# dcharatan/pixelsplat

Measured on NVIDIA H100. Metric: rendered views/sec fwd+bwd @256x256, 3 gauss/px, higher is better.
Workload: dtype f32

## Files before the change

pixelsplat_b200/csrc/ps_common.cuh:

```cuda
#pragma once
#include <cuda_runtime.h>
#include <stdint.h>

#include "../../include/pixelsplat_b200.h"

namespace ps {

constexpr int kTile = PS_TILE;
constexpr int kTilePixels = kTile * kTile;

struct Geom {
    float *depth;
    int32_t *radii;
    float2 *xy;
    float4 *conic_opacity;
    float4 *rgb;
    ushort4 *rect;
    uint8_t *clamped;
    uint32_t *tile_count;
    uint32_t *tile_start;
    uint32_t *tile_cursor;
    long long *n_instances;
    uint32_t *vis_pairs;
    float4 *cull;
};

struct ImageState {
    float *final_T;
    uint32_t *n_contrib;
    float *color;
    float4 *run_state;
    float *depth_image;
    float *run_depth;
};

// ... 66 lines not shown
    return 1.0f;
}

__device__ __forceinline__ float2 cull_extent(float a, float c, float o) {
    if (!(a > 0.0f) || !(c > 0.0f) || !(o <= 3.0e38f)) return make_float2(3.0e38f, 3.0e38f);
    if (!(o * 255.0f >= 1.0f - 1e-3f)) return make_float2(-3.0e38f, -3.0e38f);
    const float tau2 = 2.0f * (__logf(fmaxf(o * 255.0f, 1.0f)) + 0.01f);
    return make_float2(sqrtf(tau2 * a) * 1.001f + 0.01f, sqrtf(tau2 * c) * 1.001f + 0.01f);
}

constexpr uint32_t kLivePosLimit = 1u << 24;

__device__ __forceinline__ uint32_t tile_block_mask(const float4 &cr, int x0, int y0) {
    const float xl = cr.x - cr.z, xh = cr.x + cr.z, yl = cr.y - cr.w, yh = cr.y + cr.w;
    uint32_t xm = 0, m = 0;
#pragma unroll
    for (int bx = 0; bx < 2; ++bx)
        xm |= ((xh >= (float)(x0 + 8 * bx)) && (xl <= (float)(x0 + 8 * bx + 7))) ? 1u << bx : 0u;
#pragma unroll
    for (int by = 0; by < 4; ++by)
        m |= ((yh >= (float)(y0 + 4 * by)) && (yl <= (float)(y0 + 4 * by + 3))) ? xm << (2 * by) : 0u;
    return m;
}

void set_error(const char *fmt, ...);

enum Mark { kMarkFwdStart = 0, kMarkPreprocess, kMarkScatter, kMarkSort, kMarkCompositeFwd,
            kMarkBwdStart, kMarkBwdZero, kMarkCompositeBwd, kMarkPreprocessBwd, kNumMarks };
void mark(int id, cudaStream_t st);
void count_launch();

bool first_use_on_device(unsigned long long &mask);

#define PS_CUDA_CHECK(expr)                                                              \
    do {                                                                                 \
        cudaError_t _e = (expr);                                                         \
        if (_e != cudaSuccess) {                                                         \
            ps::set_error("%s failed: %s (%s:%d)", #expr, cudaGetErrorString(_e), __FILE__, __LINE__); \
            return PS_ERR_CUDA;                                                          \
        }                                                                                \
    } while (0)

#define PS_LAUNCH_CHECK(name)                                                            \
    do {                                                                                 \
        cudaError_t _e = cudaGetLastError();                                             \
        if (_e != cudaSuccess) {                                                         \
            ps::set_error("launch of %s failed: %s", name, cudaGetErrorString(_e));      \
            return PS_ERR_CUDA;                                                          \
        }                                                                                \
        ps::count_launch();                                                              \
    } while (0)

int launch_preprocess(const Dims &d, const Inputs &in, const Geom &g, cudaStream_t st);
int launch_sh_color(const Dims &d, const Inputs &in, const Geom &g, cudaStream_t st);
int launch_binning(const Dims &d, const Geom &g, unsigned long long *keys,
                   unsigned long long *keys_alt, int sort_impl, int segment_hint, cudaEvent_t scanned,
                   cudaStream_t st);
int launch_composite_forward(const Dims &d, const Inputs &in, const Geom &g,
                             const unsigned long long *keys, const uint2 *live, const ImageState &img,
                             float *out_color, const LossEpilogue &loss, const HitLists &hl, float *loss_partials,
                             cudaStream_t st);
int launch_composite_backward(const Dims &d, const Inputs &in, const Geom &g,
                              const unsigned long long *keys, const uint2 *live, const ImageState &img,
                              const float *d_color, const float *d_depth, const ViewGrads &vg,
                              const ViewGrads *records, const LossEpilogue &loss, const HitLists &hl,
                              cudaStream_t st);
// ... 17 lines not shown
```

pixelsplat_b200/csrc/raster_api.cu:

```cuda
#include <cstdarg>
#include <atomic>
#include <cstdio>
#include <cstring>
#include <mutex>

#include "ps_common.cuh"

namespace ps {

static thread_local char g_error[512] = "";

void set_error(const char *fmt, ...) {
    va_list ap;
    va_start(ap, fmt);
    vsnprintf(g_error, sizeof(g_error), fmt, ap);
    va_end(ap);
}

static bool g_timing = false;
static cudaEvent_t g_events[kNumMarks];
static bool g_events_ready = false;
static std::atomic<unsigned long long> g_launches{0};

void count_launch() { g_launches.fetch_add(1, std::memory_order_relaxed); }

static std::mutex g_once_mutex;

bool first_use_on_device(unsigned long long &mask) {
    int dev = 0;
    cudaGetDevice(&dev);
    const unsigned long long bit = 1ull << (dev & 63);
    std::lock_guard<std::mutex> lock(g_once_mutex);
    if (mask & bit) return false;
    mask |= bit;
    return true;
}

void mark(int id, cudaStream_t st) {
    if (!g_timing) return;
    if (!g_events_ready) {
        for (int i = 0; i < kNumMarks; ++i) cudaEventCreate(&g_events[i]);
        g_events_ready = true;
    }
    cudaEventRecord(g_events[id], st);
}

struct SideCtx {
    cudaStream_t side = nullptr;
    cudaEvent_t fork = nullptr, join = nullptr;
    cudaEvent_t scanned = nullptr, copied = nullptr;
    std::mutex enqueue;
};
static SideCtx g_side_ctx[64];

static int side_ready(SideCtx *&ctx) {
    int dev = 0;
    PS_CUDA_CHECK(cudaGetDevice(&dev));
    ctx = &g_side_ctx[dev & 63];
    std::lock_guard<std::mutex> lock(g_once_mutex);
    if (ctx->side) return PS_OK;
    PS_CUDA_CHECK(cudaStreamCreateWithFlags(&ctx->side, cudaStreamNonBlocking));
    PS_CUDA_CHECK(cudaEventCreateWithFlags(&ctx->fork, cudaEventDisableTiming));
    PS_CUDA_CHECK(cudaEventCreateWithFlags(&ctx->join, cudaEventDisableTiming));
    PS_CUDA_CHECK(cudaEventCreateWithFlags(&ctx->scanned, cudaEventDisableTiming));
    PS_CUDA_CHECK(cudaEventCreateWithFlags(&ctx->copied, cudaEventDisableTiming));
    return PS_OK;
}

// ... 457 lines not shown
```

pixelsplat_b200/csrc/raster_binning.cu:

```cuda
#include <cub/device/device_segmented_radix_sort.cuh>

#include "ps_common.cuh"

namespace ps {

constexpr int kScanThreads = 1024;

__global__ void __launch_bounds__(kScanThreads)
k_tile_scan(int n, const uint32_t *__restrict__ count, uint32_t *__restrict__ start,
            uint32_t *__restrict__ cursor, long long *__restrict__ n_instances) {
    __shared__ uint32_t warp_sums[32];
    __shared__ unsigned long long carry_s;
    const int tid = threadIdx.x, lane = tid & 31, warp = tid >> 5;
    if (tid == 0) carry_s = 0;
    __syncthreads();
    uint32_t cmax = 0;
    for (int base = 0; base < n; base += kScanThreads) {
        const int i = base + tid;
        const uint32_t c = i < n ? count[i] : 0u;
        cmax = max(cmax, c);
        uint32_t x = c;
#pragma unroll
        for (int o = 1; o < 32; o <<= 1) {
            const uint32_t y = __shfl_up_sync(0xffffffffu, x, o);
// ... 1 lines not shown
        }
        if (lane == 31) warp_sums[warp] = x;
        __syncthreads();
        if (warp == 0) {
            uint32_t w = warp_sums[lane];
#pragma unroll
            for (int o = 1; o < 32; o <<= 1) {
                const uint32_t y = __shfl_up_sync(0xffffffffu, w, o);
                if (lane >= o) w += y;
            }
            warp_sums[lane] = w;
        }
        __syncthreads();
        const unsigned long long carry = carry_s;
        const uint32_t warp_off = warp ? warp_sums[warp - 1] : 0u;
        const unsigned long long excl = carry + warp_off + (x - c);
        if (i < n) {
            const uint32_t e = excl > 0xffffffffull ? 0xffffffffu : (uint32_t)excl;
            start[i] = e;
            cursor[i] = e;
        }
        __syncthreads();
        if (tid == kScanThreads - 1) carry_s = carry + warp_sums[31];
        __syncthreads();
    }
    if (tid == 0) *n_instances = (long long)carry_s;
    cmax = __reduce_max_sync(0xffffffffu, cmax);
    if (lane == 0 && cmax) atomicMax(reinterpret_cast<unsigned long long *>(n_instances + 1), (unsigned long long)cmax);
}

constexpr int kScatterThreads = 256;
constexpr int kScatterMaxSmemTiles = 8192;

__global__ void __launch_bounds__(kScatterThreads)
k_scatter(Dims d, Geom geo, unsigned long long *__restrict__ keys, int use_smem) {
    extern __shared__ uint32_t s_scatter[];
    if (*geo.n_instances > d.capacity) return;
    const int vid = blockIdx.y;
    const int g = blockIdx.x * kScatterThreads + threadIdx.x;
    uint32_t *cnt = s_scatter, *base = s_scatter + d.tiles;
    uint32_t *cur = geo.tile_cursor + (size_t)vid * d.tiles;
    const size_t vg = (size_t)vid * d.P + g;
    const bool vis = g < d.P && geo.radii[vg] > 0;
    ushort4 r = make_ushort4(0, 0, 0, 0);
    unsigned long long key = 0;
    if (vis) {
        r = geo.rect[vg];
        key = ((unsigned long long)__float_as_uint(geo.depth[vg]) << 32) | (uint32_t)g;
    }
    if (!use_smem) {
        for (int ty = r.y; ty < r.w; ++ty)
            for (int tx = r.x; tx < r.z; ++tx) keys[atomicAdd(&cur[ty * d.gx + tx], 1u)] = key;
        return;
    }
    for (int i = threadIdx.x; i < d.tiles; i += kScatterThreads) cnt[i] = 0;
    __syncthreads();
    for (int ty = r.y; ty < r.w; ++ty)
        for (int tx = r.x; tx < r.z; ++tx) atomicAdd(&cnt[ty * d.gx + tx], 1u);
    __syncthreads();
    for (int i = threadIdx.x; i < d.tiles; i += kScatterThreads) {
        const uint32_t c = cnt[i];
        if (c) { base[i] = atomicAdd(&cur[i], c); cnt[i] = 0; }
    }
    __syncthreads();
    for (int ty = r.y; ty < r.w; ++ty)
        for (int tx = r.x; tx < r.z; ++tx) {
            const int t = ty * d.gx + tx;
            keys[base[t] + atomicAdd(&cnt[t], 1u)] = key;
        }
}

template <int THREADS>
__device__ void bitonic_sort_smem(unsigned long long *s_keys, int n_pad) {
    constexpr int kWarps = THREADS / 32;
    const int lane = threadIdx.x & 31, warp = threadIdx.x >> 5;
    const int chunk = max(n_pad / kWarps, 2);
    const int warps_used = n_pad / chunk;
    const int half = n_pad >> 1;
    for (int k = 2; k <= n_pad; k <<= 1) {
        int j = k >> 1;
        const bool had_global = j >= chunk;
        for (; j >= chunk; j >>= 1) {
            for (int t = threadIdx.x; t < half; t += THREADS) {
                const int i = 2 * t - (t & (j - 1));
                const int p = i + j;
                const unsigned long long a = s_keys[i], b = s_keys[p];
                const bool up = (i & k) == 0;
                if ((a > b) == up) { s_keys[i] = b; s_keys[p] = a; }
            }
            __syncthreads();
        }
        if (warp < warps_used) {
            const int base = warp * chunk;
            for (; j > 0; j >>= 1) {
                for (int t = lane; t < (chunk >> 1); t += 32) {
                    const int i = base + 2 * t - (t & (j - 1));
                    const int p = i + j;
                    const unsigned long long a = s_keys[i], b = s_keys[p];
                    const bool up = (i & k) == 0;
                    if ((a > b) == up) { s_keys[i] = b; s_keys[p] = a; }
                }
                __syncwarp();
// ... 202 lines not shown
    if (sm.misc[3]) {
        int n_pad = 2;
        while (n_pad < n) n_pad <<= 1;
        for (int i = n + tid; i < n_pad; i += kSortThreads) A[i] = ~0ull;
        __syncthreads();
        bitonic_sort_smem<kSortThreads>(A, n_pad);
    }
    for (int i = tid; i < n; i += kSortThreads) keys[s0 + i] = A[i];
    write_live_list(d, geo, A, n, seg, live, sm);
}

__global__ void __launch_bounds__(kSortThreads)
k_live_lists(Dims d, Geom geo, const unsigned long long *__restrict__ keys, unsigned long long *__restrict__ keys_alt) {
    __shared__ SortSmem sm;
    if (*geo.n_instances > d.capacity) return;
    const int seg = blockIdx.x;
    const uint32_t s0 = geo.tile_start[seg];
    write_live_list(d, geo, keys + s0, (int)geo.tile_count[seg], seg, reinterpret_cast<uint2 *>(keys_alt + s0), sm);
}

int launch_binning(const Dims &d, const Geom &g, unsigned long long *keys,
                   unsigned long long *keys_alt, int sort_impl, int segment_hint, cudaEvent_t scanned,
                   cudaStream_t st) {
    const int n_seg = d.S * d.V * d.tiles;
    k_tile_scan<<<1, kScanThreads, 0, st>>>(n_seg, g.tile_count, g.tile_start, g.tile_cursor, g.n_instances);
    PS_LAUNCH_CHECK("k_tile_scan");
    if (scanned) PS_CUDA_CHECK(cudaEventRecord(scanned, st));
    const int use_smem = d.tiles <= kScatterMaxSmemTiles;
    static unsigned long long scatter_attr_devices = 0;
    if (first_use_on_device(scatter_attr_devices)) {
        PS_CUDA_CHECK(cudaFuncSetAttribute(k_scatter, cudaFuncAttributeMaxDynamicSharedMemorySize,
                                           (int)(2 * sizeof(uint32_t) * kScatterMaxSmemTiles)));
    }
    dim3 sgrid((d.P + kScatterThreads - 1) / kScatterThreads, d.S * d.V);
    k_scatter<<<sgrid, kScatterThreads, use_smem ? 2 * sizeof(uint32_t) * d.tiles : 0, st>>>(d, g, keys, use_smem);
    PS_LAUNCH_CHECK("k_scatter");
    mark(kMarkScatter, st);

    int id_bits = 1;
    while ((1ll << id_bits) < d.P) ++id_bits;

    if (sort_impl == 1) {
        size_t temp = 0;
        cub::DoubleBuffer<unsigned long long> db(keys, keys_alt);
        PS_CUDA_CHECK(cub::DeviceSegmentedRadixSort::SortKeys(nullptr, temp, db, (int)d.capacity, n_seg,
                                                              g.tile_start, g.tile_cursor, 0, 64, st));
        void *tmp = nullptr;
        PS_CUDA_CHECK(cudaMallocAsync(&tmp, temp, st));
        PS_CUDA_CHECK(cub::DeviceSegmentedRadixSort::SortKeys(tmp, temp, db, (int)d.capacity, n_seg,
                                                              g.tile_start, g.tile_cursor, 0, 64, st));
        if (db.Current() != keys)
            PS_CUDA_CHECK(cudaMemcpyAsync(keys, db.Current(), sizeof(unsigned long long) * (size_t)d.capacity,
                                          cudaMemcpyDeviceToDevice, st));
        PS_CUDA_CHECK(cudaFreeAsync(tmp, st));
        k_live_lists<<<n_seg, kSortThreads, 0, st>>>(d, g, keys, keys_alt);
        PS_LAUNCH_CHECK("k_live_lists");
        return PS_OK;
    }

    int cap = 2048;
    if (segment_hint > 0) {
        const long long want = (long long)segment_hint + segment_hint / 4;
        while (cap < want && cap < 8192) cap <<= 1;
    }
    static unsigned long long battr_devices = 0;
    if (first_use_on_device(battr_devices)) {
        PS_CUDA_CHECK(cudaFuncSetAttribute(k_tile_sort, cudaFuncAttributeMaxDynamicSharedMemorySize,
// ... 9 lines not shown
```

pixelsplat_b200/csrc/raster_preprocess.cu:

```cuda
#include "ps_common.cuh"
#include "raster_math.cuh"

namespace ps {

constexpr int kPreThreads = 128;

__device__ __forceinline__ void warp_append(bool flag, uint32_t value, uint32_t *list, long long *counter, int lane) {
    const unsigned m = __ballot_sync(0xffffffffu, flag);
    if (m == 0u) return;
    const int leader = __ffs(m) - 1;
    unsigned long long base = 0;
    if (lane == leader)
        base = atomicAdd(reinterpret_cast<unsigned long long *>(counter), (unsigned long long)__popc(m));
    base = __shfl_sync(0xffffffffu, base, leader);
    if (flag) list[base + __popc(m & ((1u << lane) - 1u))] = value;
}

__global__ void __launch_bounds__(kPreThreads)
k_preprocess(Dims d, Inputs in, Geom geo, int use_smem_hist) {
    extern __shared__ uint32_t s_hist[];
    const int hist_n = d.V * d.tiles;
    const int scene = blockIdx.y;
    const int lane = threadIdx.x & 31;
    const int g = blockIdx.x * kPreThreads + threadIdx.x;
    const bool live = g < d.P;
    if (use_smem_hist) {
        for (int i = threadIdx.x; i < hist_n; i += kPreThreads) s_hist[i] = 0;
        __syncthreads();
    }
    const size_t sg = (size_t)scene * d.P + (live ? g : 0);
    float mx0 = 0.0f, my0 = 0.0f, mz0 = 0.0f, opacity = 0.0f;
    if (live) {
        mx0 = in.means[3 * sg + 0]; my0 = in.means[3 * sg + 1]; mz0 = in.means[3 * sg + 2];
        opacity = in.opac[sg];
    }
    const float *covp = in.cov + sg * (d.cov_layout == PS_COV_TRIU6 ? 6 : 9);
    float cov_raw[6];
    {
        float tmp[6] = {0.0f, 0.0f, 0.0f, 0.0f, 0.0f, 0.0f};
        if (live) load_cov6(covp, d.cov_layout, 1.0f, tmp);
#pragma unroll
        for (int i = 0; i < 6; ++i) cov_raw[i] = tmp[i];
    }

    for (int v = 0; v < d.V; ++v) {
        const int vid = scene * d.V + v;
        const size_t vg = (size_t)vid * d.P + (live ? g : 0);
        const float *__restrict__ vm = in.view + 16 * vid;
        const float *__restrict__ pm = in.proj + 16 * vid;
        const float sc = in.scale ? in.scale[vid] : 1.0f;
        const float px = in.scale ? mx0 * sc : mx0;
        const float py = in.scale ? my0 * sc : my0;
        const float pz = in.scale ? mz0 * sc : mz0;
        bool vis = live;
        float vz = 0.0f;
        if (vis) {
            geo.radii[vg] = 0;
            vz = vm[2] * px + vm[6] * py + vm[10] * pz + vm[14];
            vis = !(vz <= 0.2f);
        }
        if (vis) {
            const float hx = pm[0] * px + pm[4] * py + pm[8] * pz + pm[12];
            const float hy = pm[1] * px + pm[5] * py + pm[9] * pz + pm[13];
            const float hw = pm[3] * px + pm[7] * py + pm[11] * pz + pm[15];
            const float p_w = 1.0f / (hw + 0.0000001f);
            const float projx = hx * p_w, projy = hy * p_w;
            const float tanfovx = in.tanfov[2 * vid], tanfovy = in.tanfov[2 * vid + 1];
            const float focal_x = (float)d.W / (2.0f * tanfovx);
            const float focal_y = (float)d.H / (2.0f * tanfovy);
            float s6[6];
            {
                const float sc2 = sc * sc;
#pragma unroll
                for (int i = 0; i < 6; ++i) s6[i] = in.scale ? cov_raw[i] * sc2 : cov_raw[i];
            }
            Cov2D cv;
            compute_cov2d(px, py, pz, s6, vm, focal_x, focal_y, tanfovx, tanfovy, cv);
            const float det = cv.a * cv.c - cv.b * cv.b;
            vis = !(det == 0.0f);
            if (vis) {
                const float det_inv = 1.0f / det;
                const float mid = 0.5f * (cv.a + cv.c);
                const float sq = sqrtf(fmaxf(0.1f, mid * mid - det));
                const float lambda1 = mid + sq, lambda2 = mid - sq;
                const float my_radius = ceilf(3.0f * sqrtf(fmaxf(lambda1, lambda2)));
                const float pixx = ((projx + 1.0f) * (float)d.W - 1.0f) * 0.5f;
                const float pixy = ((projy + 1.0f) * (float)d.H - 1.0f) * 0.5f;
                const int r = (int)my_radius;
                const float rf = (float)r;
                const int minx = min(d.gx, max(0, (int)((pixx - rf) / (float)kTile)));
                const int miny = min(d.gy, max(0, (int)((pixy - rf) / (float)kTile)));
                const int maxx = min(d.gx, max(0, (int)((pixx + rf + (float)(kTile - 1)) / (float)kTile)));
                const int maxy = min(d.gy, max(0, (int)((pixy + rf + (float)(kTile - 1)) / (float)kTile)));
                vis = (maxx - minx) * (maxy - miny) != 0;
                if (vis) {
                    geo.depth[vg] = vz;
                    geo.radii[vg] = r;
                    geo.xy[vg] = make_float2(pixx, pixy);
                    geo.conic_opacity[vg] = make_float4(cv.c * det_inv, -cv.b * det_inv, cv.a * det_inv, opacity);
                    {
                        const float2 ext = cull_extent(cv.a, cv.c, opacity);
                        geo.cull[vg] = make_float4(pixx, pixy, ext.x, ext.y);
                    }
                    geo.rect[vg] = make_ushort4((unsigned short)minx, (unsigned short)miny,
                                                (unsigned short)maxx, (unsigned short)maxy);
                    if (d.M == 0) {
                        const float *__restrict__ col = in.sh + sg * 3;
                        const float dv = d.depth_mode ? depth_value(d.depth_mode, vz, in.scale, in.near_far, vid) : 0.0f;
                        geo.rgb[vg] = make_float4(col[0], col[1], col[2], dv);
                        geo.clamped[vg] = 0;
                    }
                    for (int ty = miny; ty < maxy; ++ty)
                        for (int tx = minx; tx < maxx; ++tx) {
                            const int t = ty * d.gx + tx;
                            if (use_smem_hist) atomicAdd(&s_hist[v * d.tiles + t], 1u);
                            else atomicAdd(&geo.tile_count[(size_t)vid * d.tiles + t], 1u);
                        }
                }
            }
        }
        warp_append(vis, (uint32_t)vg, geo.vis_pairs, geo.n_instances + 2, lane);
    }
    if (use_smem_hist) {
        __syncthreads();
        uint32_t *dst = geo.tile_count + (size_t)scene * d.V * d.tiles;
        for (int i = threadIdx.x; i < hist_n; i += kPreThreads) {
            const uint32_t c = s_hist[i];
            if (c) atomicAdd(&dst[i], c);
        }
    }
}

constexpr int kShThreads = 128;

__global__ void __launch_bounds__(kShThreads)
k_sh_color(Dims d, Inputs in, Geom geo, int row_stride) {
    extern __shared__ float s_rows[];
    const long long n = geo.n_instances[2];
    const int lane = threadIdx.x & 31, warp = threadIdx.x >> 5;
    const long long i0 = ((long long)blockIdx.x * kShThreads) + warp * 32;
    if (i0 >= n) return;
    const long long i = i0 + lane;
    const bool live = i < n;
    const uint32_t vg = live ? geo.vis_pairs[i] : 0u;
    const uint32_t vid = vg / (uint32_t)d.P, g = vg - vid * (uint32_t)d.P;
    const uint32_t scene = vid / (uint32_t)d.V;
    const size_t sg = (size_t)scene * d.P + g;
    const int sh_n = 3 * d.M;
    float *wrows = s_rows + (size_t)warp * 32 * row_stride;
    gather_rows_async(in.sh, (unsigned long long)sg, __ballot_sync(0xffffffffu, live), sh_n, wrows, row_stride, lane);
    const float sc = in.scale ? in.scale[vid] : 1.0f;
    const float m0 = in.means[3 * sg + 0], m1 = in.means[3 * sg + 1], m2 = in.means[3 * sg + 2];
    const float px = in.scale ? m0 * sc : m0, py = in.scale ? m1 * sc : m1, pz = in.scale ? m2 * sc : m2;
    const float cx = in.campos[3 * vid], cy = in.campos[3 * vid + 1], cz = in.campos[3 * vid + 2];
    const float ddx = px - cx, ddy = py - cy, ddz = pz - cz;
    const float len = sqrtf(ddx * ddx + ddy * ddy + ddz * ddz);
    const float x = ddx / len, y = ddy / len, z = ddz / len;
    gather_rows_wait();
    if (!live) return;
    const float *row = wrows + lane * row_stride;
    float acc[3] = {0.0f, 0.0f, 0.0f};
    const int M = d.M, layout = d.sh_layout;
    const float3 sa = sh_arg(d.sh_basis, x, y, z);
    const uint32_t flip = sh_flip_mask(d.sh_basis);
    sh_for_each(d.deg, sa.x, sa.y, sa.z, [&](int k, float Yk, float, float, float) {
        const float Y = sh_sign(flip, k, Yk);
#pragma unroll
        for (int ch = 0; ch < 3; ++ch) {
            const float c = row[sh_index(layout, M, k, ch)];
            acc[ch] = k == 0 ? Y * c : acc[ch] + Y * c;
        }
    });
    float rgb[3];
    uint8_t clamp_bits = 0;
#pragma unroll
    for (int ch = 0; ch < 3; ++ch) {
        const float a = acc[ch] + 0.5f;
        if (a < 0.0f) clamp_bits |= (uint8_t)(1u << ch);
        rgb[ch] = fmaxf(a, 0.0f);
    }
    const float dv = d.depth_mode ? depth_value(d.depth_mode, geo.depth[vg], in.scale, in.near_far, (int)vid) : 0.0f;
    geo.rgb[vg] = make_float4(rgb[0], rgb[1], rgb[2], dv);
    geo.clamped[vg] = clamp_bits;
}

int launch_sh_color(const Dims &d, const Inputs &in, const Geom &g, cudaStream_t st) {
    if (d.M == 0) return PS_OK;
    const int row_stride = (3 * d.M) | 1;
    const size_t smem = sizeof(float) * kShThreads * row_stride;
    static unsigned long long attr_devices = 0;
    if (first_use_on_device(attr_devices)) {
        PS_CUDA_CHECK(cudaFuncSetAttribute(k_sh_color, cudaFuncAttributeMaxDynamicSharedMemorySize, 64 * 1024));
    }
    const long long pairs = (long long)d.S * d.V * d.P;
    k_sh_color<<<(unsigned)((pairs + kShThreads - 1) / kShThreads), kShThreads, smem, st>>>(d, in, g, row_stride);
    PS_LAUNCH_CHECK("k_sh_color");
    return PS_OK;
}

int launch_preprocess(const Dims &d, const Inputs &in, const Geom &g, cudaStream_t st) {
    PS_CUDA_CHECK(cudaMemsetAsync(g.tile_count, 0, sizeof(uint32_t) * (size_t)d.S * d.V * d.tiles, st));
    PS_CUDA_CHECK(cudaMemsetAsync(g.n_instances, 0, 4 * sizeof(long long), st));
    const size_t hist_bytes = sizeof(uint32_t) * (size_t)d.V * d.tiles;
    const int use_smem = hist_bytes <= 32 * 1024;
    dim3 grid((d.P + kPreThreads - 1) / kPreThreads, d.S);
    k_preprocess<<<grid, kPreThreads, use_smem ? hist_bytes : 0, st>>>(d, in, g, use_smem);
    PS_LAUNCH_CHECK("k_preprocess");
    return PS_OK;
}

}
```

pixelsplat_b200/csrc/raster_preprocess_bwd.cu:

```cuda
#include "ps_common.cuh"
#include "raster_math.cuh"

namespace ps {

constexpr int kPreBwdThreads = 128;

__device__ __forceinline__ float *cam_row(float *ws, const Dims &d, int s, int v, long long sg0) {
    const long long w = sg0 / 32 - ((long long)s * d.P) / 32;
    return ws + ((size_t)(s * d.V + v) * cam_rows_per_view(d.P) + (size_t)w) * kCamRowFloats;
}

__device__ __forceinline__ unsigned *cam_counter(float *ws, const Dims &d, int vid) {
    return reinterpret_cast<unsigned *>(ws + (size_t)vid * cam_rows_per_view(d.P) * kCamRowFloats) + kCamEntries;
}

__device__ __forceinline__ void store_cam_partials(const float (&cam)[kCamEntries], float *cam_ws, const Dims &d,
                                                   int v, long long sg0, int rows, uint32_t scene, int lane) {
    const int s_lo = (int)(sg0 / d.P), s_hi = (int)((sg0 + rows - 1) / d.P);
    for (int s = s_lo; s <= s_hi; ++s) {
        const bool mine = (int)scene == s;
        float sum[kCamEntries];
#pragma unroll
        for (int k = 0; k < kCamEntries; ++k) {
            float x = mine ? cam[k] : 0.0f;
// ... 263 lines not shown
        }
        if constexpr (CAM) store_cam_partials(cam, cam_ws, d, v, sg0, rows, scene, lane);
    }

    if (live) {
        out.d_means[3 * sg + 0] = dmx; out.d_means[3 * sg + 1] = dmy; out.d_means[3 * sg + 2] = dmz;
        out.d_opacities[sg] = dop;
        float *dc = out.d_cov + sg * cov_n;
        if (d.cov_layout == PS_COV_TRIU6) {
#pragma unroll
            for (int i = 0; i < 6; ++i) dc[i] = dcov[i];
        } else {
            dc[0] = dcov[0]; dc[1] = dcov[1]; dc[2] = dcov[2];
            dc[3] = 0.0f; dc[4] = dcov[3]; dc[5] = dcov[4];
            dc[6] = 0.0f; dc[7] = 0.0f; dc[8] = dcov[5];
        }
        if (M == 0) {
            float *dsh = out.d_sh + sg * 3;
            dsh[0] = dcol[0]; dsh[1] = dcol[1]; dsh[2] = dcol[2];
        }
    }
    if (M > 0) {
        if (!sh_written)
            for (int c = 0; c < sh_n; ++c) grow[c] = 0.0f;
        __syncwarp();
        const float *gsrc = in_place ? wrows : wrows + (size_t)kPreBwdThreads * row_stride;
        store_rows(out.d_sh + (size_t)sg0 * sh_n, rows, sh_n, gsrc, row_stride, lane);
    }
}

constexpr int kClearThreads = 256;

__global__ void __launch_bounds__(kClearThreads) k_clear_pair_grads(Geom geo, ViewGrads vg) {
    const long long i = (long long)blockIdx.x * kClearThreads + threadIdx.x;
    if (i >= geo.n_instances[2]) return;
    const uint32_t p = geo.vis_pairs[i];
    vg.d_mean2d[p] = make_float2(0.0f, 0.0f);
    vg.d_conic[p] = make_float4(0.0f, 0.0f, 0.0f, 0.0f);
    vg.d_color[p] = make_float4(0.0f, 0.0f, 0.0f, 0.0f);
}

int launch_clear_pair_grads(const Dims &d, const Geom &g, const ViewGrads &vg, cudaStream_t st) {
    const long long pairs = (long long)d.S * d.V * d.P;
    k_clear_pair_grads<<<(unsigned)((pairs + kClearThreads - 1) / kClearThreads), kClearThreads, 0, st>>>(g, vg);
    PS_LAUNCH_CHECK("k_clear_pair_grads");
    return PS_OK;
}

constexpr int kCamBwdThreads = 128;

template <bool DEPTH>
__global__ void __launch_bounds__(kCamBwdThreads, 4)
k_camera_bwd(Dims d, Inputs in, Geom geo, ViewGrads vgr, int row_stride, float *cam_ws) {
    extern __shared__ float s_sh[];
    const int lane = threadIdx.x & 31, warp = threadIdx.x >> 5;
    const int v = (int)(blockIdx.x % (unsigned)d.V);
    const long long sp = (long long)d.S * d.P;
    const long long sg0 = (long long)(blockIdx.x / (unsigned)d.V) * kCamBwdThreads + warp * 32;
    if (sg0 >= sp) return;
    const int rows = (int)min((long long)32, sp - sg0);
    const bool live = lane < rows;
    const uint32_t sgi = (uint32_t)(live ? sg0 + lane : sg0);
    const uint32_t scene = sgi / (uint32_t)d.P, g = sgi - scene * (uint32_t)d.P;
    const size_t sg = sgi;
    const int vid = (int)scene * d.V + v;
    const size_t vg = (size_t)vid * d.P + g;
    const int M = d.M, sh_n = 3 * M;

    const bool vis = live && *geo.n_instances <= d.capacity && geo.radii[vg] > 0;
    const unsigned vis_lanes = __ballot_sync(0xffffffffu, vis);
    float cam[kCamEntries];
#pragma unroll
    for (int k = 0; k < kCamEntries; ++k) cam[k] = 0.0f;
    if (vis_lanes == 0u) {
        store_cam_partials(cam, cam_ws, d, v, sg0, rows, scene, lane);
        return;
    }
// ... 149 lines not shown
```

Before: 3140.

## Use persistent grids over visible pairs and stage preprocess inputs via cp.async

Scatter, SH colour and gradient-clear kernels now run grid-stride loops over the compacted visible-pair list, launched with a cached SM-resident grid size instead of one thread per Gaussian-view pair. This avoids launching threads for invisible pairs. Scatter also switches to iterating the visible list, handling chunks that span views by falling back to global atomics. Preprocess grows to 256 threads with 4 items each and stages means, covariances and opacities into shared memory with cp.async, trading more shared memory per CTA for fewer scattered global loads.

```diff
diff --git a/pixelsplat_b200/csrc/ps_common.cuh b/pixelsplat_b200/csrc/ps_common.cuh
--- a/pixelsplat_b200/csrc/ps_common.cuh
+++ b/pixelsplat_b200/csrc/ps_common.cuh
@@ -1,6 +1,8 @@
 #pragma once
 #include <cuda_runtime.h>
 #include <stdint.h>
+
+#include <atomic>
 
 #include "../../include/pixelsplat_b200.h"
 
@@ -133,6 +135,8 @@
 
 bool first_use_on_device(unsigned long long &mask);
 
+int resident_grid(const void *kernel, int threads, size_t smem, int per_sm, std::atomic<int> (&cache)[64], int *grid);
+
 #define PS_CUDA_CHECK(expr)                                                              \
     do {                                                                                 \
         cudaError_t _e = (expr);                                                         \
diff --git a/pixelsplat_b200/csrc/raster_api.cu b/pixelsplat_b200/csrc/raster_api.cu
--- a/pixelsplat_b200/csrc/raster_api.cu
+++ b/pixelsplat_b200/csrc/raster_api.cu
@@ -34,6 +34,21 @@
     if (mask & bit) return false;
     mask |= bit;
     return true;
+}
+
+int resident_grid(const void *kernel, int threads, size_t smem, int per_sm, std::atomic<int> (&cache)[64], int *grid) {
+    int dev = 0;
+    PS_CUDA_CHECK(cudaGetDevice(&dev));
+    int n = cache[dev & 63].load(std::memory_order_relaxed);
+    if (n == 0) {
+        int sms = 0, fit = 0;
+        PS_CUDA_CHECK(cudaDeviceGetAttribute(&sms, cudaDevAttrMultiProcessorCount, dev));
+        PS_CUDA_CHECK(cudaOccupancyMaxActiveBlocksPerMultiprocessor(&fit, kernel, threads, smem));
+        n = sms * (fit < per_sm ? (fit > 0 ? fit : 1) : per_sm);
+        cache[dev & 63].store(n, std::memory_order_relaxed);
+    }
+    *grid = n;
+    return PS_OK;
 }
 
 void mark(int id, cudaStream_t st) {
diff --git a/pixelsplat_b200/csrc/raster_binning.cu b/pixelsplat_b200/csrc/raster_binning.cu
--- a/pixelsplat_b200/csrc/raster_binning.cu
+++ b/pixelsplat_b200/csrc/raster_binning.cu
@@ -57,42 +57,51 @@
 constexpr int kScatterThreads = 256;
 constexpr int kScatterMaxSmemTiles = 8192;
 
+constexpr int kScatterCtasPerSm = 4;
+
 __global__ void __launch_bounds__(kScatterThreads)
 k_scatter(Dims d, Geom geo, unsigned long long *__restrict__ keys, int use_smem) {
     extern __shared__ uint32_t s_scatter[];
     if (*geo.n_instances > d.capacity) return;
-    const int vid = blockIdx.y;
-    const int g = blockIdx.x * kScatterThreads + threadIdx.x;
+    const long long n = geo.n_instances[2];
     uint32_t *cnt = s_scatter, *base = s_scatter + d.tiles;
-    uint32_t *cur = geo.tile_cursor + (size_t)vid * d.tiles;
-    const size_t vg = (size_t)vid * d.P + g;
-    const bool vis = g < d.P && geo.radii[vg] > 0;
-    ushort4 r = make_ushort4(0, 0, 0, 0);
-    unsigned long long key = 0;
-    if (vis) {
-        r = geo.rect[vg];
-        key = ((unsigned long long)__float_as_uint(geo.depth[vg]) << 32) | (uint32_t)g;
-    }
-    if (!use_smem) {
+    for (long long c0 = (long long)blockIdx.x * kScatterThreads; c0 < n; c0 += (long long)gridDim.x * kScatterThreads) {
+        const long long i = c0 + threadIdx.x;
+        uint32_t vid = 0;
+        ushort4 r = make_ushort4(0, 0, 0, 0);
+        unsigned long long key = 0;
+        if (i < n) {
+            const uint32_t vg = geo.vis_pairs[i];
+            vid = vg / (uint32_t)d.P;
+            r = geo.rect[vg];
+            key = ((unsigned long long)__float_as_uint(geo.depth[vg]) << 32) | (vg - vid * (uint32_t)d.P);
+        }
+        const uint32_t home = geo.vis_pairs[c0] / (uint32_t)d.P;
+        if (!use_smem || vid != home) {
+            uint32_t *cur = geo.tile_cursor + (size_t)vid * d.tiles;
+            for (int ty = r.y; ty < r.w; ++ty)
+                for (int tx = r.x; tx < r.z; ++tx) keys[atomicAdd(&cur[ty * d.gx + tx], 1u)] = key;
+            r = make_ushort4(0, 0, 0, 0);
+        }
+        if (!use_smem) continue;
+        uint32_t *cur = geo.tile_cursor + (size_t)home * d.tiles;
+        for (int t = threadIdx.x; t < d.tiles; t += kScatterThreads) cnt[t] = 0;
+        __syncthreads();
         for (int ty = r.y; ty < r.w; ++ty)
-            for (int tx = r.x; tx < r.z; ++tx) keys[atomicAdd(&cur[ty * d.gx + tx], 1u)] = key;
-        return;
-    }
-    for (int i = threadIdx.x; i < d.tiles; i += kScatterThreads) cnt[i] = 0;
-    __syncthreads();
-    for (int ty = r.y; ty < r.w; ++ty)
-        for (int tx = r.x; tx < r.z; ++tx) atomicAdd(&cnt[ty * d.gx + tx], 1u);
-    __syncthreads();
-    for (int i = threadIdx.x; i < d.tiles; i += kScatterThreads) {
-        const uint32_t c = cnt[i];
-        if (c) { base[i] = atomicAdd(&cur[i], c); cnt[i] = 0; }
-    }
-    __syncthreads();
-    for (int ty = r.y; ty < r.w; ++ty)
-        for (int tx = r.x; tx < r.z; ++tx) {
-            const int t = ty * d.gx + tx;
-            keys[base[t] + atomicAdd(&cnt[t], 1u)] = key;
-        }
+            for (int tx = r.x; tx < r.z; ++tx) atomicAdd(&cnt[ty * d.gx + tx], 1u);
+        __syncthreads();
+        for (int t = threadIdx.x; t < d.tiles; t += kScatterThreads) {
+            const uint32_t c = cnt[t];
+            if (c) { base[t] = atomicAdd(&cur[t], c); cnt[t] = 0; }
+        }
+        __syncthreads();
+        for (int ty = r.y; ty < r.w; ++ty)
+            for (int tx = r.x; tx < r.z; ++tx) {
+                const int t = ty * d.gx + tx;
+                keys[base[t] + atomicAdd(&cnt[t], 1u)] = key;
+            }
+        __syncthreads();
+    }
 }
 
 template <int THREADS>
@@ -361,7 +370,11 @@
         PS_CUDA_CHECK(cudaFuncSetAttribute(k_scatter, cudaFuncAttributeMaxDynamicSharedMemorySize,
                                            (int)(2 * sizeof(uint32_t) * kScatterMaxSmemTiles)));
     }
-    dim3 sgrid((d.P + kScatterThreads - 1) / kScatterThreads, d.S * d.V);
+    static std::atomic<int> grid_cache[64];
+    int sgrid = 0;
+    if (int rc = resident_grid((const void *)k_scatter, kScatterThreads, 2 * sizeof(uint32_t) * 1024,
+                               kScatterCtasPerSm, grid_cache, &sgrid))
+        return rc;
     k_scatter<<<sgrid, kScatterThreads, use_smem ? 2 * sizeof(uint32_t) * d.tiles : 0, st>>>(d, g, keys, use_smem);
     PS_LAUNCH_CHECK("k_scatter");
     mark(kMarkScatter, st);
diff --git a/pixelsplat_b200/csrc/raster_preprocess.cu b/pixelsplat_b200/csrc/raster_preprocess.cu
--- a/pixelsplat_b200/csrc/raster_preprocess.cu
+++ b/pixelsplat_b200/csrc/raster_preprocess.cu
@@ -3,126 +3,169 @@
 
 namespace ps {
 
-constexpr int kPreThreads = 128;
-
-__device__ __forceinline__ void warp_append(bool flag, uint32_t value, uint32_t *list, long long *counter, int lane) {
-    const unsigned m = __ballot_sync(0xffffffffu, flag);
-    if (m == 0u) return;
-    const int leader = __ffs(m) - 1;
-    unsigned long long base = 0;
-    if (lane == leader)
-        base = atomicAdd(reinterpret_cast<unsigned long long *>(counter), (unsigned long long)__popc(m));
-    base = __shfl_sync(0xffffffffu, base, leader);
-    if (flag) list[base + __popc(m & ((1u << lane) - 1u))] = value;
+constexpr int kPreThreads = 256;
+constexpr int kPreItems = 4;
+constexpr int kPreRange = kPreThreads * kPreItems;
+constexpr int kPreWarps = kPreThreads / 32;
+static_assert(kPreItems * kPreWarps == 32, "one warp scans the CTA's (item, warp) counts");
+constexpr int kPreSmemHistBytes = 32 * 1024;
+
+__device__ __forceinline__ void stage_async(float *dst, const float *__restrict__ src, int n) {
+    int i0 = 0;
+    if (((uintptr_t)src & 15) == 0) {
+        i0 = n & ~3;
+        for (int i = 4 * threadIdx.x; i < i0; i += 4 * kPreThreads) {
+            const uint32_t saddr = (uint32_t)__cvta_generic_to_shared(dst + i);
+            asm volatile("cp.async.cg.shared.global [%0], [%1], 16;" ::"r"(saddr), "l"(src + i) : "memory");
+        }
+    }
+    for (int i = i0 + threadIdx.x; i < n; i += kPreThreads) {
+        const uint32_t saddr = (uint32_t)__cvta_generic_to_shared(dst + i);
+        asm volatile("cp.async.ca.shared.global [%0], [%1], 4;" ::"r"(saddr), "l"(src + i) : "memory");
+    }
+}
+
+static size_t preprocess_smem_bytes(int cov_floats, size_t hist_bytes) {
+    return sizeof(float) * kPreRange * (3 + cov_floats + 1) + hist_bytes;
 }
 
 __global__ void __launch_bounds__(kPreThreads)
 k_preprocess(Dims d, Inputs in, Geom geo, int use_smem_hist) {
-    extern __shared__ uint32_t s_hist[];
+    extern __shared__ __align__(16) float s_pre[];
+    __shared__ uint32_t s_ballot[kPreItems * kPreWarps], s_off[kPreItems * kPreWarps];
+    const int cs = d.cov_layout == PS_COV_TRIU6 ? 6 : 9;
+    float *s_means = s_pre, *s_cov = s_pre + 3 * kPreRange, *s_opac = s_cov + cs * kPreRange;
+    uint32_t *s_hist = reinterpret_cast<uint32_t *>(s_opac + kPreRange);
     const int hist_n = d.V * d.tiles;
     const int scene = blockIdx.y;
-    const int lane = threadIdx.x & 31;
-    const int g = blockIdx.x * kPreThreads + threadIdx.x;
-    const bool live = g < d.P;
-    if (use_smem_hist) {
+    const int lane = threadIdx.x & 31, warp = threadIdx.x >> 5;
+    const int g0 = blockIdx.x * kPreRange;
+    const int n_g = min(kPreRange, d.P - g0);
+    const size_t sg0 = (size_t)scene * d.P + g0;
+    stage_async(s_means, in.means + 3 * sg0, 3 * n_g);
+    stage_async(s_cov, in.cov + cs * sg0, cs * n_g);
+    stage_async(s_opac, in.opac + sg0, n_g);
+    asm volatile("cp.async.commit_group;" ::: "memory");
+    if (use_smem_hist)
         for (int i = threadIdx.x; i < hist_n; i += kPreThreads) s_hist[i] = 0;
-        __syncthreads();
-    }
-    const size_t sg = (size_t)scene * d.P + (live ? g : 0);
-    float mx0 = 0.0f, my0 = 0.0f, mz0 = 0.0f, opacity = 0.0f;
-    if (live) {
-        mx0 = in.means[3 * sg + 0]; my0 = in.means[3 * sg + 1]; mz0 = in.means[3 * sg + 2];
-        opacity = in.opac[sg];
-    }
-    const float *covp = in.cov + sg * (d.cov_layout == PS_COV_TRIU6 ? 6 : 9);
-    float cov_raw[6];
-    {
-        float tmp[6] = {0.0f, 0.0f, 0.0f, 0.0f, 0.0f, 0.0f};
-        if (live) load_cov6(covp, d.cov_layout, 1.0f, tmp);
-#pragma unroll
-        for (int i = 0; i < 6; ++i) cov_raw[i] = tmp[i];
-    }
+    asm volatile("cp.async.wait_all;" ::: "memory");
+    __syncthreads();
 
     for (int v = 0; v < d.V; ++v) {
         const int vid = scene * d.V + v;
-        const size_t vg = (size_t)vid * d.P + (live ? g : 0);
         const float *__restrict__ vm = in.view + 16 * vid;
         const float *__restrict__ pm = in.proj + 16 * vid;
         const float sc = in.scale ? in.scale[vid] : 1.0f;
-        const float px = in.scale ? mx0 * sc : mx0;
-        const float py = in.scale ? my0 * sc : my0;
-        const float pz = in.scale ? mz0 * sc : mz0;
-        bool vis = live;
-        float vz = 0.0f;
-        if (vis) {
-            geo.radii[vg] = 0;
-            vz = vm[2] * px + vm[6] * py + vm[10] * pz + vm[14];
-            vis = !(vz <= 0.2f);
-        }
-        if (vis) {
-            const float hx = pm[0] * px + pm[4] * py + pm[8] * pz + pm[12];
-            const float hy = pm[1] * px + pm[5] * py + pm[9] * pz + pm[13];
-            const float hw = pm[3] * px + pm[7] * py + pm[11] * pz + pm[15];
-            const float p_w = 1.0f / (hw + 0.0000001f);
-            const float projx = hx * p_w, projy = hy * p_w;
-            const float tanfovx = in.tanfov[2 * vid], tanfovy = in.tanfov[2 * vid + 1];
-            const float focal_x = (float)d.W / (2.0f * tanfovx);
-            const float focal_y = (float)d.H / (2.0f * tanfovy);
-            float s6[6];
-            {
-                const float sc2 = sc * sc;
-#pragma unroll
-                for (int i = 0; i < 6; ++i) s6[i] = in.scale ? cov_raw[i] * sc2 : cov_raw[i];
-            }
-            Cov2D cv;
-            compute_cov2d(px, py, pz, s6, vm, focal_x, focal_y, tanfovx, tanfovy, cv);
-            const float det = cv.a * cv.c - cv.b * cv.b;
-            vis = !(det == 0.0f);
+#pragma unroll 1
+        for (int k = 0; k < kPreItems; ++k) {
+            const int l = k * kPreThreads + threadIdx.x;
+            const bool live = l < n_g;
+            const int g = g0 + (live ? l : 0);
+            const size_t sg = (size_t)scene * d.P + g;
+            const size_t vg = (size_t)vid * d.P + g;
+            const int ls = live ? l : 0;
+            const float mx0 = s_means[3 * ls + 0], my0 = s_means[3 * ls + 1], mz0 = s_means[3 * ls + 2];
+            const float px = in.scale ? mx0 * sc : mx0;
+            const float py = in.scale ? my0 * sc : my0;
+            const float pz = in.scale ? mz0 * sc : mz0;
+            bool vis = live;
+            float vz = 0.0f;
             if (vis) {
-                const float det_inv = 1.0f / det;
-                const float mid = 0.5f * (cv.a + cv.c);
-                const float sq = sqrtf(fmaxf(0.1f, mid * mid - det));
-                const float lambda1 = mid + sq, lambda2 = mid - sq;
-                const float my_radius = ceilf(3.0f * sqrtf(fmaxf(lambda1, lambda2)));
-                const float pixx = ((projx + 1.0f) * (float)d.W - 1.0f) * 0.5f;
-                const float pixy = ((projy + 1.0f) * (float)d.H - 1.0f) * 0.5f;
-                const int r = (int)my_radius;
-                const float rf = (float)r;
-                const int minx = min(d.gx, max(0, (int)((pixx - rf) / (float)kTile)));
-                const int miny = min(d.gy, max(0, (int)((pixy - rf) / (float)kTile)));
-                const int maxx = min(d.gx, max(0, (int)((pixx + rf + (float)(kTile - 1)) / (float)kTile)));
-                const int maxy = min(d.gy, max(0, (int)((pixy + rf + (float)(kTile - 1)) / (float)kTile)));
-                vis = (maxx - minx) * (maxy - miny) != 0;
+                geo.radii[vg] = 0;
+                vz = vm[2] * px + vm[6] * py + vm[10] * pz + vm[14];
+                vis = !(vz <= 0.2f);
+            }
+            if (vis) {
+                const float hx = pm[0] * px + pm[4] * py + pm[8] * pz + pm[12];
+                const float hy = pm[1] * px + pm[5] * py + pm[9] * pz + pm[13];
+                const float hw = pm[3] * px + pm[7] * py + pm[11] * pz + pm[15];
+                const float p_w = 1.0f / (hw + 0.0000001f);
+                const float projx = hx * p_w, projy = hy * p_w;
+                const float tanfovx = in.tanfov[2 * vid], tanfovy = in.tanfov[2 * vid + 1];
+                const float focal_x = (float)d.W / (2.0f * tanfovx);
+                const float focal_y = (float)d.H / (2.0f * tanfovy);
+                float s6[6];
+                load_cov6(s_cov + cs * ls, d.cov_layout, 1.0f, s6);
+                {
+                    const float sc2 = sc * sc;
+#pragma unroll
+                    for (int i = 0; i < 6; ++i) s6[i] = in.scale ? s6[i] * sc2 : s6[i];
+                }
+                Cov2D cv;
+                compute_cov2d(px, py, pz, s6, vm, focal_x, focal_y, tanfovx, tanfovy, cv);
+                const float det = cv.a * cv.c - cv.b * cv.b;
+                vis = !(det == 0.0f);
                 if (vis) {
-                    geo.depth[vg] = vz;
-                    geo.radii[vg] = r;
-                    geo.xy[vg] = make_float2(pixx, pixy);
-                    geo.conic_opacity[vg] = make_float4(cv.c * det_inv, -cv.b * det_inv, cv.a * det_inv, opacity);
-                    {
-                        const float2 ext = cull_extent(cv.a, cv.c, opacity);
-                        geo.cull[vg] = make_float4(pixx, pixy, ext.x, ext.y);
+                    const float opacity = s_opac[ls];
+                    const float det_inv = 1.0f / det;
+                    const float mid = 0.5f * (cv.a + cv.c);
+                    const float sq = sqrtf(fmaxf(0.1f, mid * mid - det));
+                    const float lambda1 = mid + sq, lambda2 = mid - sq;
+                    const float my_radius = ceilf(3.0f * sqrtf(fmaxf(lambda1, lambda2)));
+                    const float pixx = ((projx + 1.0f) * (float)d.W - 1.0f) * 0.5f;
+                    const float pixy = ((projy + 1.0f) * (float)d.H - 1.0f) * 0.5f;
+                    const int r = (int)my_radius;
+                    const float rf = (float)r;
+                    const int minx = min(d.gx, max(0, (int)((pixx - rf) / (float)kTile)));
+                    const int miny = min(d.gy, max(0, (int)((pixy - rf) / (float)kTile)));
+                    const int maxx = min(d.gx, max(0, (int)((pixx + rf + (float)(kTile - 1)) / (float)kTile)));
+                    const int maxy = min(d.gy, max(0, (int)((pixy + rf + (float)(kTile - 1)) / (float)kTile)));
+                    vis = (maxx - minx) * (maxy - miny) != 0;
+                    if (vis) {
+                        geo.depth[vg] = vz;
+                        geo.radii[vg] = r;
+                        geo.xy[vg] = make_float2(pixx, pixy);
+                        geo.conic_opacity[vg] = make_float4(cv.c * det_inv, -cv.b * det_inv, cv.a * det_inv, opacity);
+                        {
+                            const float2 ext = cull_extent(cv.a, cv.c, opacity);
+                            geo.cull[vg] = make_float4(pixx, pixy, ext.x, ext.y);
+                        }
+                        geo.rect[vg] = make_ushort4((unsigned short)minx, (unsigned short)miny,
+                                                    (unsigned short)maxx, (unsigned short)maxy);
+                        if (d.M == 0) {
+                            const float *__restrict__ col = in.sh + sg * 3;
+                            const float dv = d.depth_mode ? depth_value(d.depth_mode, vz, in.scale, in.near_far, vid) : 0.0f;
+                            geo.rgb[vg] = make_float4(col[0], col[1], col[2], dv);
+                            geo.clamped[vg] = 0;
+                        }
+                        for (int ty = miny; ty < maxy; ++ty)
+                            for (int tx = minx; tx < maxx; ++tx) {
+                                const int t = ty * d.gx + tx;
+                                if (use_smem_hist) atomicAdd(&s_hist[v * d.tiles + t], 1u);
+                                else atomicAdd(&geo.tile_count[(size_t)vid * d.tiles + t], 1u);
+                            }
                     }
-                    geo.rect[vg] = make_ushort4((unsigned short)minx, (unsigned short)miny,
-                                                (unsigned short)maxx, (unsigned short)maxy);
-                    if (d.M == 0) {
-                        const float *__restrict__ col = in.sh + sg * 3;
-                        const float dv = d.depth_mode ? depth_value(d.depth_mode, vz, in.scale, in.near_far, vid) : 0.0f;
-                        geo.rgb[vg] = make_float4(col[0], col[1], col[2], dv);
-                        geo.clamped[vg] = 0;
-                    }
-                    for (int ty = miny; ty < maxy; ++ty)
-                        for (int tx = minx; tx < maxx; ++tx) {
-                            const int t = ty * d.gx + tx;
-                            if (use_smem_hist) atomicAdd(&s_hist[v * d.tiles + t], 1u);
-                            else atomicAdd(&geo.tile_count[(size_t)vid * d.tiles + t], 1u);
-                        }
                 }
             }
-        }
-        warp_append(vis, (uint32_t)vg, geo.vis_pairs, geo.n_instances + 2, lane);
+            const unsigned b = __ballot_sync(0xffffffffu, vis);
+            if (lane == 0) s_ballot[k * kPreWarps + warp] = b;
+        }
+        __syncthreads();
+        if (warp == 0) {
+            const uint32_t c = (uint32_t)__popc(s_ballot[lane]);
+            uint32_t incl = c;
+#pragma unroll
+            for (int o = 1; o < 32; o <<= 1) {
+                const uint32_t y = __shfl_up_sync(0xffffffffu, incl, o);
+                if (lane >= o) incl += y;
+            }
+            unsigned long long base = 0;
+            if (lane == 31 && incl)
+                base = atomicAdd(reinterpret_cast<unsigned long long *>(geo.n_instances + 2), (unsigned long long)incl);
+            base = __shfl_sync(0xffffffffu, base, 31);
+            s_off[lane] = (uint32_t)base + incl - c;
+        }
+        __syncthreads();
+#pragma unroll
+        for (int k = 0; k < kPreItems; ++k) {
+            const unsigned b = s_ballot[k * kPreWarps + warp];
+            if ((b >> lane) & 1u)
+                geo.vis_pairs[s_off[k * kPreWarps + warp] + __popc(b & ((1u << lane) - 1u))] =
+                    (uint32_t)((size_t)vid * d.P + g0 + k * kPreThreads + threadIdx.x);
+        }
+        __syncthreads();
     }
     if (use_smem_hist) {
-        __syncthreads();
         uint32_t *dst = geo.tile_count + (size_t)scene * d.V * d.tiles;
         for (int i = threadIdx.x; i < hist_n; i += kPreThreads) {
             const uint32_t c = s_hist[i];
@@ -132,56 +175,61 @@
 }
 
 constexpr int kShThreads = 128;
+constexpr int kShCtasPerSm = 4;
 
 __global__ void __launch_bounds__(kShThreads)
 k_sh_color(Dims d, Inputs in, Geom geo, int row_stride) {
     extern __shared__ float s_rows[];
     const long long n = geo.n_instances[2];
     const int lane = threadIdx.x & 31, warp = threadIdx.x >> 5;
-    const long long i0 = ((long long)blockIdx.x * kShThreads) + warp * 32;
-    if (i0 >= n) return;
-    const long long i = i0 + lane;
-    const bool live = i < n;
-    const uint32_t vg = live ? geo.vis_pairs[i] : 0u;
-    const uint32_t vid = vg / (uint32_t)d.P, g = vg - vid * (uint32_t)d.P;
-    const uint32_t scene = vid / (uint32_t)d.V;
-    const size_t sg = (size_t)scene * d.P + g;
     const int sh_n = 3 * d.M;
     float *wrows = s_rows + (size_t)warp * 32 * row_stride;
-    gather_rows_async(in.sh, (unsigned long long)sg, __ballot_sync(0xffffffffu, live), sh_n, wrows, row_stride, lane);
-    const float sc = in.scale ? in.scale[vid] : 1.0f;
-    const float m0 = in.means[3 * sg + 0], m1 = in.means[3 * sg + 1], m2 = in.means[3 * sg + 2];
-    const float px = in.scale ? m0 * sc : m0, py = in.scale ? m1 * sc : m1, pz = in.scale ? m2 * sc : m2;
-    const float cx = in.campos[3 * vid], cy = in.campos[3 * vid + 1], cz = in.campos[3 * vid + 2];
-    const float ddx = px - cx, ddy = py - cy, ddz = pz - cz;
-    const float len = sqrtf(ddx * ddx + ddy * ddy + ddz * ddz);
-    const float x = ddx / len, y = ddy / len, z = ddz / len;
-    gather_rows_wait();
-    if (!live) return;
-    const float *row = wrows + lane * row_stride;
-    float acc[3] = {0.0f, 0.0f, 0.0f};
     const int M = d.M, layout = d.sh_layout;
-    const float3 sa = sh_arg(d.sh_basis, x, y, z);
     const uint32_t flip = sh_flip_mask(d.sh_basis);
-    sh_for_each(d.deg, sa.x, sa.y, sa.z, [&](int k, float Yk, float, float, float) {
-        const float Y = sh_sign(flip, k, Yk);
-#pragma unroll
-        for (int ch = 0; ch < 3; ++ch) {
-            const float c = row[sh_index(layout, M, k, ch)];
-            acc[ch] = k == 0 ? Y * c : acc[ch] + Y * c;
-        }
-    });
-    float rgb[3];
-    uint8_t clamp_bits = 0;
-#pragma unroll
-    for (int ch = 0; ch < 3; ++ch) {
-        const float a = acc[ch] + 0.5f;
-        if (a < 0.0f) clamp_bits |= (uint8_t)(1u << ch);
-        rgb[ch] = fmaxf(a, 0.0f);
-    }
-    const float dv = d.depth_mode ? depth_value(d.depth_mode, geo.depth[vg], in.scale, in.near_far, (int)vid) : 0.0f;
-    geo.rgb[vg] = make_float4(rgb[0], rgb[1], rgb[2], dv);
-    geo.clamped[vg] = clamp_bits;
+    for (long long i0 = ((long long)blockIdx.x * kShThreads) + warp * 32; i0 < n;
+         i0 += (long long)gridDim.x * kShThreads) {
+        const long long i = i0 + lane;
+        const bool live = i < n;
+        const uint32_t vg = live ? geo.vis_pairs[i] : 0u;
+        const uint32_t vid = vg / (uint32_t)d.P, g = vg - vid * (uint32_t)d.P;
+        const uint32_t scene = vid / (uint32_t)d.V;
+        const size_t sg = (size_t)scene * d.P + g;
+        gather_rows_async(in.sh, (unsigned long long)sg, __ballot_sync(0xffffffffu, live), sh_n, wrows, row_stride,
+                          lane);
+        const float sc = in.scale ? in.scale[vid] : 1.0f;
+        const float m0 = in.means[3 * sg + 0], m1 = in.means[3 * sg + 1], m2 = in.means[3 * sg + 2];
+        const float px = in.scale ? m0 * sc : m0, py = in.scale ? m1 * sc : m1, pz = in.scale ? m2 * sc : m2;
+        const float cx = in.campos[3 * vid], cy = in.campos[3 * vid + 1], cz = in.campos[3 * vid + 2];
+        const float ddx = px - cx, ddy = py - cy, ddz = pz - cz;
+        const float len = sqrtf(ddx * ddx + ddy * ddy + ddz * ddz);
+        const float x = ddx / len, y = ddy / len, z = ddz / len;
+        gather_rows_wait();
+        if (live) {
+            const float *row = wrows + lane * row_stride;
+            float acc[3] = {0.0f, 0.0f, 0.0f};
+            const float3 sa = sh_arg(d.sh_basis, x, y, z);
+            sh_for_each(d.deg, sa.x, sa.y, sa.z, [&](int k, float Yk, float, float, float) {
+                const float Y = sh_sign(flip, k, Yk);
+#pragma unroll
+                for (int ch = 0; ch < 3; ++ch) {
+                    const float c = row[sh_index(layout, M, k, ch)];
+                    acc[ch] = k == 0 ? Y * c : acc[ch] + Y * c;
+                }
+            });
+            float rgb[3];
+            uint8_t clamp_bits = 0;
+#pragma unroll
+            for (int ch = 0; ch < 3; ++ch) {
+                const float a = acc[ch] + 0.5f;
+                if (a < 0.0f) clamp_bits |= (uint8_t)(1u << ch);
+                rgb[ch] = fmaxf(a, 0.0f);
+            }
+            const float dv = d.depth_mode ? depth_value(d.depth_mode, geo.depth[vg], in.scale, in.near_far, (int)vid) : 0.0f;
+            geo.rgb[vg] = make_float4(rgb[0], rgb[1], rgb[2], dv);
+            geo.clamped[vg] = clamp_bits;
+        }
+        __syncwarp();
+    }
 }
 
 int launch_sh_color(const Dims &d, const Inputs &in, const Geom &g, cudaStream_t st) {
@@ -192,8 +240,12 @@
     if (first_use_on_device(attr_devices)) {
         PS_CUDA_CHECK(cudaFuncSetAttribute(k_sh_color, cudaFuncAttributeMaxDynamicSharedMemorySize, 64 * 1024));
     }
-    const long long pairs = (long long)d.S * d.V * d.P;
-    k_sh_color<<<(unsigned)((pairs + kShThreads - 1) / kShThreads), kShThreads, smem, st>>>(d, in, g, row_stride);
+    static std::atomic<int> grid_cache[64];
+    int grid = 0;
+    if (int rc = resident_grid((const void *)k_sh_color, kShThreads, sizeof(float) * kShThreads * (75 | 1),
+                               kShCtasPerSm, grid_cache, &grid))
+        return rc;
+    k_sh_color<<<grid, kShThreads, smem, st>>>(d, in, g, row_stride);
     PS_LAUNCH_CHECK("k_sh_color");
     return PS_OK;
 }
@@ -202,9 +254,15 @@
     PS_CUDA_CHECK(cudaMemsetAsync(g.tile_count, 0, sizeof(uint32_t) * (size_t)d.S * d.V * d.tiles, st));
     PS_CUDA_CHECK(cudaMemsetAsync(g.n_instances, 0, 4 * sizeof(long long), st));
     const size_t hist_bytes = sizeof(uint32_t) * (size_t)d.V * d.tiles;
-    const int use_smem = hist_bytes <= 32 * 1024;
-    dim3 grid((d.P + kPreThreads - 1) / kPreThreads, d.S);
-    k_preprocess<<<grid, kPreThreads, use_smem ? hist_bytes : 0, st>>>(d, in, g, use_smem);
+    const int use_smem = hist_bytes <= kPreSmemHistBytes;
+    static unsigned long long attr_devices = 0;
+    if (first_use_on_device(attr_devices)) {
+        PS_CUDA_CHECK(cudaFuncSetAttribute(k_preprocess, cudaFuncAttributeMaxDynamicSharedMemorySize,
+                                           (int)preprocess_smem_bytes(9, kPreSmemHistBytes)));
+    }
+    const size_t smem = preprocess_smem_bytes(d.cov_layout == PS_COV_TRIU6 ? 6 : 9, use_smem ? hist_bytes : 0);
+    dim3 grid((d.P + kPreRange - 1) / kPreRange, d.S);
+    k_preprocess<<<grid, kPreThreads, smem, st>>>(d, in, g, use_smem);
     PS_LAUNCH_CHECK("k_preprocess");
     return PS_OK;
 }
diff --git a/pixelsplat_b200/csrc/raster_preprocess_bwd.cu b/pixelsplat_b200/csrc/raster_preprocess_bwd.cu
--- a/pixelsplat_b200/csrc/raster_preprocess_bwd.cu
+++ b/pixelsplat_b200/csrc/raster_preprocess_bwd.cu
@@ -319,17 +319,20 @@
 constexpr int kClearThreads = 256;
 
 __global__ void __launch_bounds__(kClearThreads) k_clear_pair_grads(Geom geo, ViewGrads vg) {
-    const long long i = (long long)blockIdx.x * kClearThreads + threadIdx.x;
-    if (i >= geo.n_instances[2]) return;
-    const uint32_t p = geo.vis_pairs[i];
-    vg.d_mean2d[p] = make_float2(0.0f, 0.0f);
-    vg.d_conic[p] = make_float4(0.0f, 0.0f, 0.0f, 0.0f);
-    vg.d_color[p] = make_float4(0.0f, 0.0f, 0.0f, 0.0f);
-}
-
-int launch_clear_pair_grads(const Dims &d, const Geom &g, const ViewGrads &vg, cudaStream_t st) {
-    const long long pairs = (long long)d.S * d.V * d.P;
-    k_clear_pair_grads<<<(unsigned)((pairs + kClearThreads - 1) / kClearThreads), kClearThreads, 0, st>>>(g, vg);
+    const long long n = geo.n_instances[2];
+    for (long long i = (long long)blockIdx.x * kClearThreads + threadIdx.x; i < n; i += (long long)gridDim.x * kClearThreads) {
+        const uint32_t p = geo.vis_pairs[i];
+        vg.d_mean2d[p] = make_float2(0.0f, 0.0f);
+        vg.d_conic[p] = make_float4(0.0f, 0.0f, 0.0f, 0.0f);
+        vg.d_color[p] = make_float4(0.0f, 0.0f, 0.0f, 0.0f);
+    }
+}
+
+int launch_clear_pair_grads(const Dims &, const Geom &g, const ViewGrads &vg, cudaStream_t st) {
+    static std::atomic<int> grid_cache[64];
+    int grid = 0;
+    if (int rc = resident_grid((const void *)k_clear_pair_grads, kClearThreads, 0, 8, grid_cache, &grid)) return rc;
+    k_clear_pair_grads<<<grid, kClearThreads, 0, st>>>(g, vg);
     PS_LAUNCH_CHECK("k_clear_pair_grads");
     return PS_OK;
 }
```

Result: faster. 3229, median of 6 (+2.8%).
